# codebits1001/CET-driven-simulation-for-3D-printing-AM-KMC-Approach

Hardware: AMD Instinct MI355X
Metric: kmc_events_per_sec (higher is better)
Workload: dtype f64

## Files before the change

cet-driven-simulation-for-3d-printing-am-kmc-approach_amd/cetkmc/_lib.py:

```python
import ctypes as C
import glob
import os
import subprocess

_HERE = os.path.dirname(os.path.abspath(__file__))
CSRC = os.path.join(os.path.dirname(_HERE), "csrc")
INCLUDE = os.path.join(os.path.dirname(os.path.dirname(_HERE)), "include")
SO_PATH = os.path.join(CSRC, "libcetkmc_hip.so")


def sources():
    return sorted(glob.glob(os.path.join(CSRC, "*.hip")) + glob.glob(os.path.join(CSRC, "*.hpp")) +
                  glob.glob(os.path.join(INCLUDE, "*.h")))


HIPCC_FLAGS = ["--offload-arch=gfx950", "-O3", "-std=c++17", "-fPIC", "-shared", "-ffp-contract=off",
               "-fno-fast-math", "-I/opt/rocm/include"]


class Params(C.Structure):
    _fields_ = [
        ("nu", C.c_double), ("nu_dep", C.c_double), ("E_b", C.c_double * 3), ("E_diff", C.c_double * 3),
        ("kT", C.c_double), ("T_melt", C.c_double), ("I0", C.c_double), ("delta_T_c", C.c_double),
        ("K_nuc", C.c_double), ("beta_imp_nuc", C.c_double), ("max_imp_frac", C.c_double),
# ... 99 lines not shown
        ("n_bins", C.c_int32), ("pad", C.c_int32), ("gb_edges", C.POINTER(C.c_double)), ("pole_edges", C.POINTER(C.c_double)),
        ("axis", C.c_double * 3),
    ]


class SolidInfo(C.Structure):
    _fields_ = [("n_new", C.c_int64), ("n_cleared", C.c_int64), ("n_recorded", C.c_int64)]


class SolidArgs(C.Structure):
    _fields_ = [("qscale", C.c_double * 4)]


class SolidRec(C.Structure):
    _fields_ = [("n_rec", C.c_int64), ("n_bad", C.c_int64), ("n_cooling", C.c_int64), ("stamp_sum", C.c_int64),
                ("stamp_min", C.c_int64), ("stamp_max", C.c_int64), ("q", C.c_int64 * 4)]


STRUCT_MIRRORS = {"params": Params, "event": Event, "sweep_info": SweepInfo, "run_args": RunArgs, "run_result": RunResult,
                  "super_args": SuperArgs, "counters": Counters, "host_comm": HostComm, "ens_args": EnsArgs,
                  "ens_analysis": EnsAnalysis, "front_stats": FrontStats, "layer_rec": LayerRec,
                  "texture_args": TextureArgs, "grain_rec": GrainRec, "solid_info": SolidInfo, "solid_args": SolidArgs,
                  "solid_rec": SolidRec}

_P = C.POINTER
PROTOTYPES = {
    "cetkmc_last_error": (C.c_char_p, []),
    "cetkmc_abi_version": (C.c_int, []),
    "cetkmc_source_hash": (C.c_char_p, []),
    "cetkmc_struct_size": (C.c_int, [C.c_char_p]),
    "cetkmc_dirty_offset": (C.c_int, [C.c_int, C.c_int]),
    "cetkmc_stale_row": (C.c_int, [C.c_int, _P(C.c_int), _P(C.c_int), C.c_int, C.c_int]),
    "cetkmc_stale_rows": (C.c_int, [C.c_int, _P(C.c_int), _P(C.c_int), C.c_int, C.c_void_p]),
    "cetkmc_device_count": (C.c_int, [_P(C.c_int)]),
    "cetkmc_create": (C.c_int, [_P(Params), C.c_int, C.c_int, _P(C.c_int), _P(C.c_void_p)]),
    "cetkmc_get_unique_id": (C.c_int, [C.c_char_p]),
    "cetkmc_create_rank": (C.c_int, [_P(Params), C.c_int, C.c_int, C.c_int, C.c_int, C.c_char_p, _P(C.c_void_p)]),
    "cetkmc_create_rank_host": (C.c_int, [_P(Params), C.c_int, C.c_int, C.c_int, C.c_int, _P(HostComm), _P(C.c_void_p)]),
    "cetkmc_destroy": (C.c_int, [C.c_void_p]),
    "cetkmc_set_params": (C.c_int, [C.c_void_p, _P(Params)]),
    "cetkmc_sync": (C.c_int, [C.c_void_p]),
    "cetkmc_set_option": (C.c_int, [C.c_void_p, C.c_char_p, C.c_int64]),
    "cetkmc_owned_planes": (C.c_int, [C.c_void_p, _P(C.c_int), _P(C.c_int)]),
    "cetkmc_upload": (C.c_int, [C.c_void_p, C.c_void_p, C.c_void_p, C.c_void_p, C.c_void_p, C.c_void_p]),
    "cetkmc_download": (C.c_int, [C.c_void_p, C.c_void_p, C.c_void_p, C.c_void_p, C.c_void_p, C.c_void_p]),
    "cetkmc_upload_planes": (C.c_int, [C.c_void_p, C.c_int, C.c_int, C.c_void_p, C.c_void_p, C.c_void_p, C.c_void_p, C.c_void_p]),
    "cetkmc_download_planes": (C.c_int, [C.c_void_p, C.c_int, C.c_int, C.c_void_p, C.c_void_p, C.c_void_p, C.c_void_p, C.c_void_p]),
    "cetkmc_set_defects": (C.c_int, [C.c_void_p, C.c_void_p]),
    "cetkmc_set_prev_state": (C.c_int, [C.c_void_p, C.c_void_p]),
    "cetkmc_thermal_cet": (C.c_int, [C.c_void_p, C.c_double, C.c_int]),
    "cetkmc_thermal_laser": (C.c_int, [C.c_void_p, C.c_double, C.c_void_p, C.c_int, C.c_int]),
    "cetkmc_rate_sweep": (C.c_int, [C.c_void_p, _P(SweepInfo)]),
    "cetkmc_select": (C.c_int, [C.c_void_p, C.c_double, _P(Event)]),
    "cetkmc_apply": (C.c_int, [C.c_void_p, _P(Event), C.c_double, C.c_double, C.c_int]),
    "cetkmc_enumerate_events": (C.c_int, [C.c_void_p, C.c_void_p, C.c_int64, _P(C.c_int64)]),
    "cetkmc_row_sums": (C.c_int, [C.c_void_p, C.c_void_p, C.c_void_p]),
    "cetkmc_run_steps": (C.c_int, [C.c_void_p, _P(RunArgs), _P(RunResult), C.c_void_p, C.c_void_p, C.c_void_p]),
    "cetkmc_stage_inputs": (C.c_int, [C.c_void_p, _P(RunArgs)]),
    "cetkmc_run_supersteps": (C.c_int, [C.c_void_p, _P(SuperArgs), _P(RunResult), C.c_void_p, C.c_void_p, C.c_void_p, C.c_void_p]),
    "cetkmc_get_counters": (C.c_int, [C.c_void_p, _P(Counters), C.c_int]),
    "cetkmc_cluster": (C.c_int, [C.c_void_p, C.c_double, _P(C.c_int64)]),
    "cetkmc_cluster_stats": (C.c_int, [C.c_void_p, C.c_int64, C.c_void_p, C.c_void_p, C.c_void_p]),
    "cetkmc_cluster_labels": (C.c_int, [C.c_void_p, C.c_void_p]),
    "cetkmc_species_counts": (C.c_int, [C.c_void_p, C.c_void_p]),
    "cetkmc_gather_species": (C.c_int, [C.c_void_p, C.c_int, C.c_void_p, C.c_void_p, C.c_int64, _P(C.c_int64)]),
    "cetkmc_set_defects_sparse": (C.c_int, [C.c_void_p, C.c_void_p, C.c_int64]),
# ... 123 lines not shown
```

cet-driven-simulation-for-3d-printing-am-kmc-approach_amd/csrc/cetkmc_hip.hip:

```cpp
#include <dlfcn.h>
#include <hip/hip_runtime.h>
#include <hip/hip_ext.h>
#include <rccl/rccl.h>

#include <algorithm>
#include <chrono>
#include <cmath>
#include <cstdint>
#include <climits>
#include <cstdio>
#include <cstring>
#include <map>
#include <mutex>
#include <string>
#include <type_traits>
#include <vector>

#include "kernels.hpp"
#include "cluster.hpp"
#include "superstep.hpp"
#include "ensemble.hpp"
#include "front.hpp"
#include "layer.hpp"
#include "texture.hpp"
// ... 78 lines not shown
#define NCCLCHK(expr)                                                                             \
    do {                                                                                          \
        ncclResult_t r_ = (expr);                                                                 \
        if (r_ != ncclSuccess)                                                                    \
            return fail(std::string(#expr) + ": " + g_rccl.GetErrorString(r_));                   \
    } while (0)

struct Slab {
    SlabView v{};
    uint8_t* prev = nullptr;
    double* Tbuf[2] = {nullptr, nullptr};
    double* vvalbuf[2] = {nullptr, nullptr};
    double* depbuf[2] = {nullptr, nullptr};
    size_t nS = 0, nT = 0, nC = 0;
};

struct Handle {
    cetkmc_params p{};
    KParams kp{};
    int L = 0, Pk = 1, PB = 1, RJ = 0, pitchS = 0, pitchT = 0, pitchC = 0;
    int dev = 0;
    hipStream_t stream = nullptr, stream2 = nullptr;
    std::vector<Slab> slabs;
    SlabView* d_views[2] = {nullptr, nullptr};
    int cur = 0;
    int G = 1, my_first = 0;
    int own_i0 = 0, own_i1 = 0;
    BlockEnt* d_blocks = nullptr;
    cetkmc_event* d_events_all = nullptr;
    StepState* d_ss = nullptr;
    int* d_dirty = nullptr;
    PendRec* d_pend = nullptr;
    int apply_in_sweep = 1;
    bool pend_live = false;
    BatchCfg pend_cfg{};
    double* d_ktab = nullptr;
    KParams* d_kp = nullptr;
    void* d_scratch = nullptr;
    size_t scratch_bytes = 0;
    int* d_flag = nullptr;
    double* d_qtop = nullptr;
    double *d_u_pick = nullptr, *d_u_defect = nullptr, *d_u_np = nullptr, *d_q = nullptr, *d_log_total = nullptr;
    cetkmc_event* d_log_event = nullptr;
    int64_t* d_log_nev = nullptr;
    size_t cap_steps = 0, cap_np = 0, cap_q = 0;
    char* pin_in = nullptr; size_t pin_in_cap = 0;
    char* pin_out = nullptr; size_t pin_out_cap = 0;
    struct { bool valid = false, has_defect = false; int64_t step0 = 0, n_steps = 0, np_cap = 0, n_q = 0; int thermal_mode = 0; } staged;
    ncclComm_t comm = nullptr;
    int rank = 0, nranks = 1;
    bool swept = false;
    int sweep_auto = 1;
    int sweep_variant = 1;
    bool table_fresh = false;
    bool ifc_fresh = false;
    int ifc_every_step = 0;
    int thermal_variant = 1;
    int thermal_general = 0;
    int therm_ni = THERM_NI;
    int therm_ni16 = THERM16_NI;
    int thermal_rpt = 2;
    int thermal_kt = 256;
    int thermal_tiles16 = 1;
    int ifc_blocks = 64;
    int ifc_block = 256;
    size_t shmem_stream = 0;
// ... 459 lines not shown
    HIPCHK(hipMemcpyAsync(buf, host, per * h->nranks, hipMemcpyHostToDevice, h->stream));
    HIPCHK(hipStreamSynchronize(h->stream));
    return 0;
}
int comm_allgather(Handle* h, void* buf, size_t per)
{
    CHK(comm_stamp(h));
    CHK(comm_allgather_raw(h, buf, per));
    return comm_stamp(h);
}

int launch_dirty_rows(Handle* h, hipEvent_t ev_a, hipEvent_t ev_b)
{
    if (ev_a) HIPCHK(hipEventRecord(ev_a, h->stream));
    for (size_t s = 0; s < h->slabs.size(); ++s) {
        SlabView v = view_of(h, (int)s);
        const StreamArgs sa = stream_args(h, v);
        const int* dl = h->d_dirty;
        int* pc = h->d_dirty + 1 + DIRTY_MAX;
        const StepState* ss = h->d_ss;
        with_rows(row_shape(h), [&](auto hw, auto ch2) {
            with_flag(h->sweep_variant == 1 || h->sweep_variant >= 3, [&](auto tab) {
                launch(k_rows_eval<tab.value, hw.value, ch2.value>, dim3(24), dim3(256), 0, h->stream, nullptr, nullptr, sa, dl, ss, h->d_blocks, pc);
            });
        });
    }
    if (ev_b) HIPCHK(hipEventRecord(ev_b, h->stream));
    HIPCHK(hipGetLastError());
    if (multi_rank(h)) CHK(comm_allgather(h, h->d_blocks, (size_t)3 * (h->L / h->nranks) * sizeof(BlockEnt)));
    h->swept = true;
    return 0;
}

int launch_sweep(Handle* h, bool batch, hipEvent_t ev_a = nullptr, hipEvent_t ev_b = nullptr, bool long_list = false,
                 hipEvent_t ev_pre = nullptr, hipEvent_t ev_post = nullptr)
{
    ++h->cnt.sweeps;
    for (auto& sl : h->slabs) h->cnt.alg_bytes_sweep += (int64_t)9 * sl.v.nloc * h->L * h->L;
    if (ev_pre) HIPCHK(hipEventRecord(ev_pre, h->stream));
    const int TR = SWEEP_TJ + 4;
    const size_t shmem0 = (size_t)((5 * TR * h->pitchS + 15) & ~15) + 225 * sizeof(double);
    const StepState* ss = batch ? h->d_ss : nullptr;
    const int njt = (h->L + SWEEP_TJ - 1) / SWEEP_TJ;
    if (h->sweep_variant >= 1) {
        if (h->pend_live && (!h->table_fresh || !h->ifc_fresh)) return fail("internal: rate table / interface sums stale under a pending event");
        CHK(ensure_table(h, h->stream, ss));
        if (!h->ifc_fresh || h->ifc_every_step) {
            CHK(launch_interface(h, batch, h->stream, long_list));
            ++h->cnt.interface_launches;
            h->ifc_fresh = true;
        }
    }
    const bool ext = ev_a && ev_b && !ev_pre && h->slabs.size() == 1 && h->sweep_variant >= 1;
    const hipEvent_t xa = ext ? ev_a : nullptr, xb = ext ? ev_b : nullptr;
    if (ev_a && !ext) HIPCHK(hipEventRecord(ev_a, h->stream));
    const int sv = (h->sweep_auto && h->sweep_variant == 1 && h->L <= 128) ? 4 : h->sweep_variant;
    const RowShape rs = row_shape(h);
    for (size_t s = 0; s < h->slabs.size(); ++s) {
        SlabView v = view_of(h, (int)s);
        const StreamArgs sa = stream_args(h, v);
        if (sv == 4) {
            with_rows(rs, [&](auto hw, auto ch2) {
                launch(k_sweep_plane<hw.value, ch2.value>, dim3((unsigned)v.nloc), dim3(1024), plane_shmem(h->L), h->stream, xa, xb, sa, ss, h->d_blocks);
            });
        } else if (sv == 3) {
            const int ipp = rs.hw ? (h->L + 1) / 2 : h->L;
            const int64_t n_items = (int64_t)ipp * v.nloc;
            const dim3 g((unsigned)((n_items + 4 * TABLE_IPW - 1) / (4 * TABLE_IPW)));
            with_rows(rs, [&](auto hw, auto ch2) {
                launch(k_sweep_table<hw.value, ch2.value>, g, dim3(256), 0, h->stream, xa, xb, sa, ss);
            });
        } else if (h->sweep_variant >= 1 && h->pend_live) {
            ApplyArgs X{h->kp, (const SlabView*)h->d_views[h->cur], h->d_pend, h->d_ss, h->pend_cfg, (const double*)h->d_u_defect,
                        (const double*)h->d_u_np, (const double*)h->d_ktab, h->d_log_total, h->d_log_event, h->d_log_nev};
            launch(k_sweep_stream_apply<true, 1, false>, dim3(sa.group_count * njt + 1), dim3(256), h->shmem_stream, h->stream, xa, xb, sa, h->d_ss, X);
        } else if (h->sweep_variant >= 1) {
            auto go = [&](auto k) { launch(k, dim3(sa.group_count * njt), dim3(256), h->shmem_stream, h->stream, xa, xb, sa, ss); };
            if (h->sweep_variant == 1) with_stream_kernel<true>(rs, go); else with_stream_kernel<false>(rs, go);
        } else {
            hipLaunchKernelGGL(k_sweep_simple, dim3(v.nloc * njt), dim3(256), shmem0, h->stream, h->kp, v, h->d_ktab, ss);
        }
    }
    if (ev_b && !ext) HIPCHK(hipEventRecord(ev_b, h->stream));
    if (sv != 4)
        for (size_t s = 0; s < h->slabs.size(); ++s) {
            SlabView v = view_of(h, (int)s);
            hipLaunchKernelGGL(k_plane_reduce, dim3(3 * v.nloc), dim3(64), 0, h->stream, v, h->d_blocks, ss);
        }
    HIPCHK(hipGetLastError());
    if (multi_rank(h)) CHK(comm_allgather(h, h->d_blocks, (size_t)3 * (h->L / h->nranks) * sizeof(BlockEnt)));
    if (ev_post) HIPCHK(hipEventRecord(ev_post, h->stream));
    h->swept = true;
    return 0;
}

int launch_select(Handle* h, const BatchCfg& cfg, double r_direct, int info_only)
{
    hipLaunchKernelGGL(k_select, dim3(1), dim3(256), 0, h->stream, h->kp, (const SlabView*)h->d_views[h->cur],
                       (int)h->slabs.size(), h->L, h->PB, (const BlockEnt*)h->d_blocks, h->d_ss, cfg,
                       (const double*)h->d_u_pick, r_direct, (const double*)h->d_ktab,
                       h->d_events_all + h->my_first, info_only, h->sweep_variant >= 1 ? 1 : 0);
    HIPCHK(hipGetLastError());
    if (multi_rank(h) && !info_only) CHK(comm_allgather(h, h->d_events_all, sizeof(cetkmc_event)));
    return 0;
}

int launch_select_apply(Handle* h, const BatchCfg& cfg, int eval_touched, int* dirty, int64_t cur_hint)
{
// ... 381 lines not shown
const char* cetkmc_last_error(void) { return g_err.c_str(); }
int cetkmc_abi_version(void) { return CETKMC_ABI_VERSION; }
#ifndef CETKMC_SRC_HASH
#define CETKMC_SRC_HASH "unknown"
#endif
static const char g_src_hash[] = "cetkmc-source-hash=" CETKMC_SRC_HASH;
const char* cetkmc_source_hash(void) { return g_src_hash + 19; }

int cetkmc_struct_size(const char* name)
{
    if (!name) return -1;
#define SZ(n, t) if (!strcmp(name, n)) return (int)sizeof(t)
    SZ("params", cetkmc_params); SZ("event", cetkmc_event); SZ("sweep_info", cetkmc_sweep_info);
    SZ("run_args", cetkmc_run_args); SZ("run_result", cetkmc_run_result); SZ("super_args", cetkmc_super_args);
    SZ("counters", cetkmc_counters); SZ("host_comm", cetkmc_host_comm); SZ("ens_args", cetkmc_ens_args); SZ("ens_analysis", cetkmc_ens_analysis);
    SZ("front_stats", struct cetkmc_front_stats); SZ("layer_rec", struct cetkmc_layer_rec); SZ("texture_args", struct cetkmc_texture_args);
    SZ("grain_rec", struct cetkmc_grain_rec);
    SZ("solid_info", struct cetkmc_solid_info); SZ("solid_args", struct cetkmc_solid_args); SZ("solid_rec", struct cetkmc_solid_rec);
#undef SZ
    return -1;
}

int cetkmc_dirty_offset(int di, int dj) { return dirty_offset(di, dj) ? 1 : 0; }
static StaleEv stale_ev_host(int type, const int pos[2], const int target[2])
{
    StaleEv se;
    se.type = type; se.pi = pos[0]; se.pj = pos[1]; se.ti = target[0]; se.tj = target[1];
    return se;
}
int cetkmc_stale_row(int type, const int pos[2], const int target[2], int gi, int j)
{
    return stale_row(stale_ev_host(type, pos, target), gi, j) ? 1 : 0;
}
int cetkmc_stale_rows(int type, const int pos[2], const int target[2], int L, int rows[][2])
{
    const StaleEv se = stale_ev_host(type, pos, target);
    int n = 0;
    for (int c = 0; c < STALE_CAND; ++c) {
        int gi, j;
        if (!stale_candidate(se, L, c, gi, j)) continue;
        if (n < PATCH_MAX) { rows[n][0] = gi; rows[n][1] = j; }
        ++n;
    }
    return n;
}

int cetkmc_device_count(int* n)
{
    if (!n) return fail("null argument");
    int c = 0;
    hipError_t e = hipGetDeviceCount(&c);
    if (e != hipSuccess) { *n = 0; return fail(std::string("hipGetDeviceCount: ") + hipGetErrorString(e)); }
    *n = c;
    return 0;
}

int cetkmc_create(const cetkmc_params* p, int L, int n_slabs, const int* device_ids, void** handle)
{
    if (n_slabs < 1) return fail("n_slabs must be >= 1");
    int dev = device_ids ? device_ids[0] : 0;
    for (int s = 1; s < n_slabs && device_ids; ++s)
        if (device_ids[s] != dev)
            return fail("in-process slabs must share one device; multi-GPU runs use one process per GPU (cetkmc_create_rank)");
    if (n_slabs > 1 && L / n_slabs < 2) return fail("each slab needs at least 2 planes");
    std::vector<std::pair<int, int>> ranges;
    int base = L / n_slabs, rem = L % n_slabs, at = 0;
// ... 65 lines not shown
{
    Handle* h = (Handle*)handle;
    if (!h || !p) return fail("null argument");
    HIPCHK(hipSetDevice(h->dev));
    h->p = *p; h->kp = make_kparams(*p);
    h->swept = false; h->table_fresh = false; h->ifc_fresh = false;
    return upload_ktab(h);
}

int cetkmc_set_option(void* handle, const char* key, int64_t value)
{
    Handle* h = (Handle*)handle;
    if (!h || !key) return fail("null argument");
    if (!strcmp(key, "sweep_variant")) {
        if (value < 0 || value > 4) return fail("sweep_variant must be 0 (simple), 1 (streaming + rate table, default), 2 (streaming, recompute), 3 (census-free table sweep) or 4 (census-free, one block per plane, block sums in the same launch)");
        h->sweep_variant = (int)value;
        h->sweep_auto = 0;
        h->swept = false; h->table_fresh = false; h->ifc_fresh = false;
        return 0;
    }
    if (!strcmp(key, "interface_every_step")) { h->ifc_every_step = value ? 1 : 0; h->ifc_fresh = false; return 0; }
    if (!strcmp(key, "thermal_planes_per_block")) {
        if (value < 1 || value > 64) return fail("thermal_planes_per_block must be 1..64");
        h->therm_ni = (int)value;
        return 0;
    }
    if (!strcmp(key, "thermal_planes_per_block16")) {
        if (value < 1 || value > 64) return fail("thermal_planes_per_block16 must be 1..64");
        h->therm_ni16 = (int)value;
        return 0;
    }
    if (!strcmp(key, "thermal_lookahead")) { h->thermal_ahead = value ? 1 : 0; return 0; }
    if (!strcmp(key, "apply_in_sweep")) { h->apply_in_sweep = value ? 1 : 0; return 0; }
    if (!strcmp(key, "thermal_table")) { h->thermal_table = value ? 1 : 0; return 0; }
    if (!strcmp(key, "reserve_batch")) {
        if (value < 0 || value > (1 << 22)) return fail("reserve_batch out of range");
        HIPCHK(hipSetDevice(h->dev));
        h->staged.valid = false;
        const size_t n = (size_t)value;
        CHK(reserve_steps(h, n));
        CHK(grow(&h->d_u_np, &h->cap_np, 2 * n + 2 + (size_t)h->L * h->L));
        CHK(grow(&h->d_q, &h->cap_q, (n / 20 + 2) * (size_t)h->L * h->L));
        CHK(grow_pinned(&h->pin_in, &h->pin_in_cap, 2 * n * 8 + (2 * n + 2) * 8 + std::min<size_t>(PIN_SMALL_MAX, (n / 20 + 2) * (size_t)h->L * h->L * 8)));
        CHK(grow_pinned(&h->pin_out, &h->pin_out_cap, 64 + n * (16 + sizeof(cetkmc_event)) + h->slabs.size() * sizeof(int)));
        return reserve_events(h, std::max<int64_t>(7 * std::min<int64_t>(value, 256), value <= 64 ? 2 * value : 2 * (value / 8 + 1)));
    }
    if (!strcmp(key, "thermal_variant")) {
        if (value < 0 || value > 5) return fail("thermal_variant must be 0 (simple), 1 (marching, default: 16-row tiles, 2 rows per thread), 2 (marching, general kernel only), 3 (16-row tiles, 4 rows per thread), 4 (8-row tiles) or 5 (16-row x 128-column tiles)");
        h->thermal_general = value == 2 ? 1 : 0;
        h->thermal_tiles16 = value == 4 ? 0 : 1;
        h->thermal_rpt = value == 3 ? 4 : 2;
        h->thermal_kt = value == 5 ? 128 : 256;
        if (value >= 2) value = 1;
        h->thermal_variant = (int)value;
        return 0;
    }
    return fail(std::string("unknown option ") + key);
}

int cetkmc_sync(void* handle)
{
    Handle* h = (Handle*)handle;
    if (!h) return fail("null handle");
    HIPCHK(hipStreamSynchronize(h->stream));
    return 0;
}
// ... 1897 lines not shown
```

cet-driven-simulation-for-3d-printing-am-kmc-approach_amd/csrc/kernels.hpp:

```cpp
#pragma once
#include "voxel.hpp"
#include "../../include/cetkmc.h"

namespace cetkmc {

struct BlockEnt { double sum; int64_t cnt; };

struct StepState {
    int64_t cur;
    int32_t status;
    int32_t pad0;
    int64_t np_pos;
    int64_t nuc_count;
    double  total;
    int64_t n_events;
    int64_t n_dep;
    double  min_margin;
};

template <class S> __device__ __forceinline__ const auto& ens_rep(unsigned r, const S& sel) { return sel.reps[r]; }
template <class S> __device__ __forceinline__ int ens_rel(const S& sel) { return sel.rel; }
template <class S> __device__ __forceinline__ unsigned ens_nz(const S& sel) { return (unsigned)sel.nz; }
template <class S> __device__ __forceinline__ int64_t ens_stride(const S& sel) { return sel.stride; }
template <class S> __device__ __forceinline__ const long long* ens_offs(const S& sel) { return sel.offs; }
// ... 555 lines not shown
            {
                load_vals<TAB, HW>(A, li, j0 + row_of(1), lane, 0, nxt);
                const int r = row_of(0);
                auto rowp = [&](int d, int dj) { return (const uint8_t*)smem + so[d + 2] + (r + 2 + dj) * pitchC + KOFFC; };
                sweep_row<TAB, HW, CH2, SK>(A, rowp, li, lp, j0 + r, top, lane, cur, sw);
            }
            {
#ifdef CETKMC_NO_TAIL_PREFETCH
                if (more)
#endif
                load_vals<TAB, HW>(A, min(li + 1, lp1 + 1), j0 + row_of(0), lane, 0, cur);
                const int r = row_of(1);
                auto rowp = [&](int d, int dj) { return (const uint8_t*)smem + so[d + 2] + (r + 2 + dj) * pitchC + KOFFC; };
                sweep_row<TAB, HW, CH2, SK>(A, rowp, li, lp, j0 + r, top, lane, nxt, sw);
            }
        }
#ifdef CETKMC_NO_TAIL_PREFETCH
        if (more)
#endif
        store_slab(li + 3);
        __syncthreads();
    };
    if (NP == 1) {
#pragma unroll 1
        for (int lp = lp0; lp < lp1; lp += 2) {
            plane(lp, va, vb);
            if (lp + 1 < lp1) plane(lp + 1, vb, va);
        }
    } else {
#pragma unroll 1
        for (int lp = lp0; lp < lp1; ++lp) plane(lp, va, vb);
    }
}
template <bool TAB, bool HW, int NPF, bool CH2>
__global__ __launch_bounds__(256) CETKMC_SWEEP_ATTR void k_sweep_stream(StreamArgs A, const StepState* __restrict__ ss)
{
    if (ss && ss->status) return;
    extern __shared__ __attribute__((aligned(16))) unsigned char smem[];
    sweep_stream_tile<TAB, HW, NPF, CH2>(A, blockIdx.x, smem);
}

__device__ __forceinline__ uint2 load_cls8(const StreamArgs& A, int li, int jrow, int sl, int m)
{
    const int k0 = min((m << 9) + 8 * sl, A.pitchT - 8);
    const int jr = min(jrow, A.L - 1);
    return *reinterpret_cast<const uint2*>(A.cls + ((int64_t)li * A.RJ + (jr + 2)) * A.pitchC + KOFFC + k0);
}
template <bool HW, bool CH2>
__device__ __forceinline__ void table_row(const StreamArgs& A, int li, int lp, int jrow, bool top, int lane, const double (&v0)[8],
                                          uint2 own0, double* lds_sum = nullptr, int* lds_cnt = nullptr )
{
    static_assert(!(HW && CH2), "half-wave rows have one chunk");
    const int L = A.L;
    const int sl = HW ? (lane & 31) : lane;
    constexpr int nch = CH2 ? 2 : 1;
    double r0 = 0.0, r1 = 0.0, r2 = 0.0;
    int nE_a = 0, nE_b = 0, nD_a = 0, nD_b = 0;
    int cI = 0;
    bool any_ifc = false;
#pragma unroll
    for (int m = 0; m < nch; ++m) {
        const int k0 = (m << 9) + 8 * sl;
        const bool active = jrow < L && k0 < L;
        double v[8], ev[8];
        uint2 own = own0;
        if (m == 0) {
#pragma unroll
            for (int q = 0; q < 8; ++q) v[q] = v0[q];
        } else {
            load_vals<true, HW>(A, li, jrow, lane, m, v);
            own = load_cls8(A, li, jrow, sl, m);
        }
        if (!active) own = make_uint2(0u, 0u);
        const uint2 E = make_uint2(own.x & 0x01010101u, own.y & 0x01010101u);
        const uint2 Aat = make_uint2((own.x >> 1) & 0x01010101u, (own.y >> 1) & 0x01010101u);
        const uint2 c6 = make_uint2((own.x >> 2) & 0x3F3F3F3Fu, (own.y >> 2) & 0x3F3F3F3Fu);
#pragma unroll
        for (int h = 0; h < 8; ++h) ev[h] = mask_f64(v[h], h < 4 ? E.x : E.y, 8 * (h & 3));
        const uint2 cE = make_uint2(c6.x & (E.x * 255u), c6.y & (E.y * 255u));
        const uint2 cA = make_uint2(c6.x & (Aat.x * 255u), c6.y & (Aat.y * 255u));
        const bool diff_here = __any((cA.x | cA.y) != 0u);
        double dv[8];
#pragma unroll
// ... 20 lines not shown
        r2 = (m == 0) ? s2 : r2 + s2;
        double s1 = 0.0;
        if (diff_here) s1 = wave_tree_sum_h<HW>(tree8(dv));
        r1 = (m == 0) ? s1 : r1 + s1;
        if (top) {
            double dp[8];
#pragma unroll
            for (int q = 0; q < 8; ++q) dp[q] = 0.0;
            if (active) {
                const double2* src = reinterpret_cast<const double2*>(A.dep_val + (int64_t)jrow * A.pitchT + k0);
#pragma unroll
                for (int q = 0; q < 4; ++q) { const double2 t = src[q]; dp[2 * q] = t.x; dp[2 * q + 1] = t.y; }
            }
#pragma unroll
            for (int h = 0; h < 8; ++h) {
                const bool keep = (((h < 4 ? E.x : E.y) >> (8 * (h & 3))) & 1u) && finite_d(dp[h]);
                dp[h] = keep ? dp[h] : 0.0;
                const unsigned long long bm = __ballot(keep);
                if (HW) { nD_a += __popc((unsigned)bm); nD_b += __popc((unsigned)(bm >> 32)); }
                else nD_a += __popcll(bm);
            }
            const double s0 = wave_tree_sum_h<HW>(tree8(dp));
            r0 = (m == 0) ? s0 : r0 + s0;
        }
    }
    int n2 = HW ? ((lane & 32) ? nE_b : nE_a) : nE_a;
    const int n0 = HW ? ((lane & 32) ? nD_b : nD_a) : nD_a;
    int n1 = 0;
    if (any_ifc) {
        const int packed = wave_sum_i_h<HW>(cI);
        n2 += packed & 0xFFFF;
        n1 = packed >> 16;
    }
    if (sl == 0 && jrow < L) {
        const int64_t o = (int64_t)lp * 3 * L + jrow;
        A.rowsum[o] = r0; A.rowsum[o + L] = r1; A.rowsum[o + 2 * (int64_t)L] = r2;
        A.rowcnt[o] = n0; A.rowcnt[o + L] = n1; A.rowcnt[o + 2 * (int64_t)L] = n2;
        if (lds_sum) {
            lds_sum[jrow] = r0; lds_sum[L + jrow] = r1; lds_sum[2 * L + jrow] = r2;
            lds_cnt[jrow] = n0; lds_cnt[L + jrow] = n1; lds_cnt[2 * L + jrow] = n2;
        }
    }
}

#ifndef CETKMC_TABLE_IPW
#define CETKMC_TABLE_IPW 8
#endif
constexpr int TABLE_IPW = CETKMC_TABLE_IPW;
template <bool HW, bool CH2>
__global__ __launch_bounds__(256) CETKMC_SWEEP_ATTR void k_sweep_table(StreamArgs A, const StepState* __restrict__ ss)
{
    if (ss && ss->status) return;
    const int tid = threadIdx.x, lane = tid & 63, w = tid >> 6;
    const int L = A.L;
    const int ipp = HW ? (L + 1) >> 1 : L;
    const int n_items = ipp * A.nloc;
    int b = blockIdx.x;
    if ((gridDim.x & 7) == 0) b = (b & 7) * (int)(gridDim.x >> 3) + (b >> 3);
    int item = b * 4 * TABLE_IPW + w;
    if (item >= n_items) return;
    int lp = item / ipp, jp = item - lp * ipp;
    const int sl = HW ? (lane & 31) : lane;
    auto jrow_of = [&](int jpair) { return HW ? 2 * jpair + (lane >> 5) : jpair; };
#ifdef CETKMC_TABLE_DEPTH2
    double va[8], vb[8], vc[8];
    uint2 ca, cb, cc;
    auto advance = [&](int& lpx, int& jpx) { jpx += 4; while (jpx >= ipp) { jpx -= ipp; ++lpx; } };
    int lp1 = lp, jp1 = jp;
    advance(lp1, jp1);
    const bool has1 = item + 4 < n_items;
    load_vals<true, HW>(A, lp + 2, jrow_of(jp), lane, 0, va);
    ca = load_cls8(A, lp + 2, jrow_of(jp), sl, 0);
    load_vals<true, HW>(A, (has1 ? lp1 : lp) + 2, jrow_of(has1 ? jp1 : jp), lane, 0, vb);
    cb = load_cls8(A, (has1 ? lp1 : lp) + 2, jrow_of(has1 ? jp1 : jp), sl, 0);
    int done = 0;
    auto step = [&](double (&cur)[8], uint2& ccur, double (&far)[8], uint2& cfar) {
        int lp2 = lp, jp2 = jp;
        advance(lp2, jp2);
        int lp3 = lp2, jp3 = jp2;
        advance(lp3, jp3);
        const bool more = (done + 2 < TABLE_IPW) && (item + 8 < n_items);
        load_vals<true, HW>(A, (more ? lp3 : lp) + 2, jrow_of(more ? jp3 : jp), lane, 0, far);
        cfar = load_cls8(A, (more ? lp3 : lp) + 2, jrow_of(more ? jp3 : jp), sl, 0);
        table_row<HW, CH2>(A, lp + 2, lp, jrow_of(jp), A.gi0 + lp == L - 1, lane, cur, ccur);
        item += 4; lp = lp2; jp = jp2; ++done;
    };
#pragma unroll 1
    while (true) {
        step(va, ca, vc, cc);
        if (done >= TABLE_IPW || item >= n_items) break;
        step(vb, cb, va, ca);
        if (done >= TABLE_IPW || item >= n_items) break;
        step(vc, cc, vb, cb);
        if (done >= TABLE_IPW || item >= n_items) break;
    }
#else
    double va[8], vb[8];
    uint2 ca, cb;
    load_vals<true, HW>(A, lp + 2, jrow_of(jp), lane, 0, va);
    ca = load_cls8(A, lp + 2, jrow_of(jp), sl, 0);
    auto step = [&](double (&cur)[8], uint2& ccur, double (&nxt)[8], uint2& cnxt, bool last) {
        int lp2 = lp, jp2 = jp + 4;
        while (jp2 >= ipp) { jp2 -= ipp; ++lp2; }
        const bool more = !last && (item + 4 < n_items);
        const int lpn = more ? lp2 : lp, jpn = more ? jp2 : jp;
        load_vals<true, HW>(A, lpn + 2, jrow_of(jpn), lane, 0, nxt);
        cnxt = load_cls8(A, lpn + 2, jrow_of(jpn), sl, 0);
        table_row<HW, CH2>(A, lp + 2, lp, jrow_of(jp), A.gi0 + lp == L - 1, lane, cur, ccur);
        item += 4; lp = lp2; jp = jp2;
    };
#pragma unroll 1
    for (int t = 0; t < TABLE_IPW; t += 2) {
        step(va, ca, vb, cb, false);
        if (item >= n_items) break;
        step(vb, cb, va, ca, t + 2 >= TABLE_IPW);
        if (item >= n_items) break;
    }
#endif
}

template <bool HW, bool CH2, class... E>
__global__ __launch_bounds__(1024) CETKMC_SWEEP_ATTR void k_sweep_plane(StreamArgs A, const StepState* __restrict__ ss, BlockEnt* __restrict__ blocks, E... ens)
{
    if constexpr (sizeof...(E) > 0) {
        const auto& e = ens_rep(blockIdx.y, ens...);
        A = e.sa[ens_rel(ens...)]; ss = e.ss; blocks = e.blocks;
    }
    if (ss && ss->status) return;
    extern __shared__ __attribute__((aligned(16))) unsigned char smem[];
    const int tid = threadIdx.x, lane = tid & 63, w = tid >> 6;
    const int L = A.L;
    double* lds_sum = reinterpret_cast<double*>(smem);
    int* lds_cnt = reinterpret_cast<int*>(lds_sum + 3 * L);
    const int ipp = HW ? (L + 1) >> 1 : L;
    int lp = blockIdx.x;
    if ((gridDim.x & 7) == 0) lp = (lp & 7) * (int)(gridDim.x >> 3) + (lp >> 3);
    const int sl = HW ? (lane & 31) : lane;
    auto jrow_of = [&](int jpair) { return HW ? 2 * jpair + (lane >> 5) : jpair; };
    const bool top = A.gi0 + lp == L - 1;
    int jp = w;
    if (jp < ipp) {
        double va[8], vb[8];
        uint2 ca, cb;
        load_vals<true, HW>(A, lp + 2, jrow_of(jp), lane, 0, va);
        ca = load_cls8(A, lp + 2, jrow_of(jp), sl, 0);
        auto step = [&](double (&cur)[8], uint2& ccur, double (&nxt)[8], uint2& cnxt) {
            const int jpn = (jp + 16 < ipp) ? jp + 16 : jp;
            load_vals<true, HW>(A, lp + 2, jrow_of(jpn), lane, 0, nxt);
            cnxt = load_cls8(A, lp + 2, jrow_of(jpn), sl, 0);
            table_row<HW, CH2>(A, lp + 2, lp, jrow_of(jp), top, lane, cur, ccur, lds_sum, lds_cnt);
// ... 981 lines not shown
    for (int q = threadIdx.x; q < (int)(sizeof(SlabView) / 8); q += blockDim.x)
        reinterpret_cast<uint64_t*>(Sl)[q] = reinterpret_cast<const uint64_t*>(X.slabs)[q];
    __syncthreads();
    apply_batch_body<PEND_EB>(*Pl, Sl, 1, A.L, &X.pend->ev, 1, X.ss, X.cfg, X.u_defect, X.u_np, X.log_total, X.log_event, X.log_nev,
                              X.ktab_g, 1, nullptr, &X.pend->carry);
#ifdef CETKMC_SEL_STAMPS
    if (threadIdx.x == 0) g_pend_stamps[1] = g_sel_stamps[10];
#endif
    __builtin_amdgcn_fence(__ATOMIC_RELEASE, "agent");
    __syncthreads();
    __builtin_amdgcn_fence(__ATOMIC_ACQUIRE, "agent");
    PEND_STAMP(2);
    const StaleEv se = stale_ev_of(X.pend->ev);
    const int lane = threadIdx.x & 63, w = __builtin_amdgcn_readfirstlane((int)(threadIdx.x >> 6)), L = A.L;
    int cgi = 0, cj = 0;
    unsigned long long m = __ballot(lane < STALE_CAND && stale_candidate(se, L, lane, cgi, cj));
    for (int k = w; k > 0; --k) m &= m - 1;
    while (m) {
        int gi, j;
        stale_candidate_row(se, __builtin_ctzll(m), gi, j);
        const int lp = gi - A.gi0, li = lp + 2;
        const int jrow = (HW && lane >= 32) ? L_INACTIVE : j;
        double v0[8];
        load_vals<true, HW>(A, li, jrow, lane, 0, v0);
        table_row<HW, CH2>(A, li, lp, jrow, gi == L - 1, lane, v0, load_cls8(A, li, jrow, HW ? (lane & 31) : lane, 0));
        for (int k = 4; k > 0; --k) m &= m - 1;
    }
#ifdef CETKMC_SEL_STAMPS
    __syncthreads();
    PEND_STAMP(3);
#endif
}

template <bool HW, int NPF, bool CH2>
__global__ __launch_bounds__(256) __attribute__((amdgpu_waves_per_eu(5))) void k_sweep_stream_apply(StreamArgs A,
                                                                                                    const StepState* __restrict__ ss,
                                                                                                    ApplyArgs X)
{
    if (ss->status) return;
    extern __shared__ __attribute__((aligned(16))) unsigned char smem[];
    if (blockIdx.x != 0) {
        const int b = (int)blockIdx.x - 1;
        const StaleEv se = stale_ev_of(X.pend->ev);
        int ibr, jt;
        stream_tile_of(A, b, ibr, jt);
        const int g0 = A.gi0 + (A.group_first + ibr) * STREAM_NI, j0 = jt * SWEEP_TJ;
        auto meets = [&](int ci, int cj) {
            return ci + 2 >= g0 && ci - 2 < g0 + STREAM_NI && cj + 2 >= j0 && cj - 2 < j0 + SWEEP_TJ;
        };
        if (se.type >= 0 && (meets(se.pi, se.pj) || (se.type == EV_DIFF && meets(se.ti, se.tj))))
            sweep_stream_tile<true, HW, NPF, CH2, true>(A, b, smem, stale_win(se));
        else
            sweep_stream_tile<true, HW, NPF, CH2>(A, b, smem);
#ifdef CETKMC_SEL_STAMPS
        if (threadIdx.x == 0) atomicMax(&g_pend_stamps[4], (unsigned long long)wall_clock64());
#endif
        return;
    }
    sweep_apply_block<HW, CH2>(A, X, smem);
}

__global__ __launch_bounds__(64) void k_apply_direct(KParams P, const SlabView* __restrict__ slabs, int nslabs, cetkmc_event ev,
                                                     int make_defect, StepState* ss, const double* __restrict__ ktab_g)
{
    if (threadIdx.x == 0) {
        if (ev.type == EV_NUC) ss->nuc_count += 1;
        apply_event(slabs, nslabs, ev, make_defect);
    }
    __syncthreads();
    apply_touch(P, slabs, nslabs, ktab_g, ev, threadIdx.x, 0, blockDim.x);
}

__global__ void k_empty() {}

template <class... E>
__global__ void k_batch_reset(StepState* ss, E... ens)
{
    if constexpr (sizeof...(E) > 0) {
        const auto& e = ens_rep(blockIdx.x, ens...);
        ss = e.ss;
        if (!e.active) { ss->cur = 0; ss->status = 1; ss->np_pos = 0; ss->min_margin = 1.0; return; }
    }
    ss->cur = 0; ss->status = 0; ss->np_pos = 0; ss->min_margin = 1.0;
}

struct ThermalCfg {
// ... 564 lines not shown
```

include/cetkmc.h:

```cpp
#ifndef CETKMC_H
#define CETKMC_H

#include <stdint.h>

#ifdef __cplusplus
extern "C" {
#endif

#define CETKMC_ABI_VERSION 1

typedef struct cetkmc_params {
    double nu;
    double nu_dep;
    double E_b[3];
    double E_diff[3];
    double kT;
    double T_melt;
    double I0;
    double delta_T_c;
    double K_nuc;
    double beta_imp_nuc;
    double max_imp_frac;
    double rate_threshold;
    double anisotropy;
// ... 68 lines not shown
    int32_t thermal_mode;
    double  thermal_dt;
    const double* q_planes;
    int64_t n_q;
    int32_t use_latent;
    int32_t null_events;
} cetkmc_super_args;

typedef struct cetkmc_counters {
    int64_t steps;
    int64_t sweeps;
    int64_t incremental_steps;
    int64_t thermal_updates;
    int64_t supersteps;
    int64_t bytes_h2d, bytes_d2h;
    int64_t alg_bytes_sweep, alg_bytes_thermal;
    int64_t profiled_steps;
    double  ms_thermal, ms_interface , ms_sweep, ms_dirty_rows, ms_reduce, ms_select_apply;
    int64_t alg_bytes_table;
    int64_t table_updates;
    int64_t interface_launches;
    double  ms_comm;
    int64_t comm_calls;
    int64_t deferred_steps;
} cetkmc_counters;

const char* cetkmc_last_error(void);
int cetkmc_abi_version(void);
const char* cetkmc_source_hash(void);
int cetkmc_struct_size(const char* name);
int cetkmc_dirty_offset(int di, int dj);
int cetkmc_stale_row(int type, const int pos[2], const int target[2], int gi, int j);
int cetkmc_stale_rows(int type, const int pos[2], const int target[2], int L, int rows[][2]);
int cetkmc_device_count(int* n);

int cetkmc_create(const cetkmc_params* p, int L, int n_slabs, const int* device_ids, void** handle);
int cetkmc_get_unique_id(char out[128]);
int cetkmc_create_rank(const cetkmc_params* p, int L, int rank, int nranks, int device_id,
                       const char unique_id[128], void** handle);
typedef int (*cetkmc_allgather_fn)(void* user, const void* send, void* recv, int64_t nbytes);
typedef int (*cetkmc_exchange_fn)(void* user, int lo, int hi, const void* send_lo, void* recv_lo, const void* send_hi,
                                  void* recv_hi, int64_t nbytes);
typedef struct cetkmc_host_comm {
    cetkmc_allgather_fn allgather;
    cetkmc_exchange_fn exchange;
    void* user;
} cetkmc_host_comm;
int cetkmc_create_rank_host(const cetkmc_params* p, int L, int rank, int nranks, int device_id, const cetkmc_host_comm* hc,
                            void** handle);
int cetkmc_destroy(void* handle);
int cetkmc_set_params(void* handle, const cetkmc_params* p);
int cetkmc_sync(void* handle);
int cetkmc_set_option(void* handle, const char* key, int64_t value);
int cetkmc_owned_planes(void* handle, int* i0, int* i1);

int cetkmc_upload(void* handle, const int64_t* state, const double* theta, const double* phi,
                  const double* T, const int64_t* defects);
int cetkmc_download(void* handle, int64_t* state, double* theta, double* phi, double* T,
                    int64_t* defects);
int cetkmc_upload_planes(void* handle, int i_begin, int i_end, const uint8_t* state,
                         const double* theta, const double* phi, const double* T,
                         const uint8_t* defects);
int cetkmc_download_planes(void* handle, int i_begin, int i_end, uint8_t* state, double* theta,
                           double* phi, double* T, uint8_t* defects);
int cetkmc_set_defects(void* handle, const uint8_t* mask);
int cetkmc_set_prev_state(void* handle, const int64_t* prev_state);
// ... 143 lines not shown
```

Before: 17020.

## Use census-free table tiles in the pending-event sweep-apply launch

Adds a table-tile sweep path that assigns row items to waves in a flat, interleaved order with double-buffered loads. It reads from the rate table instead of using ring-shaped shared-memory stream tiles. The fused sweep+apply kernel uses this path by default for single-slab, single-rank runs with L>128 and half-wave rows, skipping rowsum writes for rows made stale by the pending event. The aim is to drop shared-memory staging and the per-tile stale-window checks, and to spread work across more, smaller blocks. The risk is lower reuse of neighbor data, and the path only runs at particular shapes.

```diff
diff --git a/cet-driven-simulation-for-3d-printing-am-kmc-approach_amd/cetkmc/_lib.py b/cet-driven-simulation-for-3d-printing-am-kmc-approach_amd/cetkmc/_lib.py
--- a/cet-driven-simulation-for-3d-printing-am-kmc-approach_amd/cetkmc/_lib.py
+++ b/cet-driven-simulation-for-3d-printing-am-kmc-approach_amd/cetkmc/_lib.py
@@ -155,6 +155,7 @@
     "cetkmc_dirty_offset": (C.c_int, [C.c_int, C.c_int]),
     "cetkmc_stale_row": (C.c_int, [C.c_int, _P(C.c_int), _P(C.c_int), C.c_int, C.c_int]),
     "cetkmc_stale_rows": (C.c_int, [C.c_int, _P(C.c_int), _P(C.c_int), C.c_int, C.c_void_p]),
+    "cetkmc_table_tile_of": (C.c_int, [C.c_int, C.c_int, C.c_int]),
     "cetkmc_device_count": (C.c_int, [_P(C.c_int)]),
     "cetkmc_create": (C.c_int, [_P(Params), C.c_int, C.c_int, _P(C.c_int), _P(C.c_void_p)]),
     "cetkmc_get_unique_id": (C.c_int, [C.c_char_p]),
diff --git a/cet-driven-simulation-for-3d-printing-am-kmc-approach_amd/csrc/cetkmc_hip.hip b/cet-driven-simulation-for-3d-printing-am-kmc-approach_amd/csrc/cetkmc_hip.hip
--- a/cet-driven-simulation-for-3d-printing-am-kmc-approach_amd/csrc/cetkmc_hip.hip
+++ b/cet-driven-simulation-for-3d-printing-am-kmc-approach_amd/csrc/cetkmc_hip.hip
@@ -134,6 +134,7 @@
     int* d_dirty = nullptr;
     PendRec* d_pend = nullptr;
     int apply_in_sweep = 1;
+    int fused_tiles = 1;
     bool pend_live = false;
     BatchCfg pend_cfg{};
     double* d_ktab = nullptr;
@@ -659,6 +660,12 @@
     return 0;
 }
 
+bool table_tiles(const Handle* h, int level)
+{
+    return h->fused_tiles >= level && h->slabs.size() == 1 && !multi_rank(h) && h->L > 128 && row_shape(h).hw;
+}
+size_t apply_shmem() { return ((sizeof(KParams) + 15) & ~(size_t)15) + sizeof(SlabView); }
+
 int launch_sweep(Handle* h, bool batch, hipEvent_t ev_a = nullptr, hipEvent_t ev_b = nullptr, bool long_list = false,
                  hipEvent_t ev_pre = nullptr, hipEvent_t ev_post = nullptr)
 {
@@ -700,7 +707,12 @@
         } else if (h->sweep_variant >= 1 && h->pend_live) {
             ApplyArgs X{h->kp, (const SlabView*)h->d_views[h->cur], h->d_pend, h->d_ss, h->pend_cfg, (const double*)h->d_u_defect,
                         (const double*)h->d_u_np, (const double*)h->d_ktab, h->d_log_total, h->d_log_event, h->d_log_nev};
-            launch(k_sweep_stream_apply<true, 1, false>, dim3(sa.group_count * njt + 1), dim3(256), h->shmem_stream, h->stream, xa, xb, sa, h->d_ss, X);
+            if (table_tiles(h, 1))
+                launch(k_sweep_stream_apply<true, 1, false, true>, dim3(table_tile_count(h->L, v.nloc, true) + 1), dim3(256), apply_shmem(), h->stream, xa, xb, sa, h->d_ss, X);
+            else
+                launch(k_sweep_stream_apply<true, 1, false>, dim3(sa.group_count * njt + 1), dim3(256), h->shmem_stream, h->stream, xa, xb, sa, h->d_ss, X);
+        } else if (h->sweep_variant == 1 && table_tiles(h, 2)) {
+            launch(k_sweep_stream<true, true, 1, false, true>, dim3(table_tile_count(h->L, v.nloc, true)), dim3(256), 0, h->stream, xa, xb, sa, ss);
         } else if (h->sweep_variant >= 1) {
             auto go = [&](auto k) { launch(k, dim3(sa.group_count * njt), dim3(256), h->shmem_stream, h->stream, xa, xb, sa, ss); };
             if (h->sweep_variant == 1) with_stream_kernel<true>(rs, go); else with_stream_kernel<false>(rs, go);
@@ -1148,6 +1160,11 @@
 {
     return stale_row(stale_ev_host(type, pos, target), gi, j) ? 1 : 0;
 }
+int cetkmc_table_tile_of(int L, int gi, int j)
+{
+    if (L <= 128 || L > 256 || gi < 0 || gi >= L || j < 0 || j >= L) return -1;
+    return table_tile_of(L, true, gi, j);
+}
 int cetkmc_stale_rows(int type, const int pos[2], const int target[2], int L, int rows[][2])
 {
     const StaleEv se = stale_ev_host(type, pos, target);
@@ -1279,6 +1296,11 @@
     }
     if (!strcmp(key, "thermal_lookahead")) { h->thermal_ahead = value ? 1 : 0; return 0; }
     if (!strcmp(key, "apply_in_sweep")) { h->apply_in_sweep = value ? 1 : 0; return 0; }
+    if (!strcmp(key, "fused_tiles")) {
+        if (value < 0 || value > 2) return fail("fused_tiles must be 0 (ring tiles), 1 (census-free tiles in the launch that applies a pending event, default) or 2 (in the plain streaming launch at that shape as well)");
+        h->fused_tiles = (int)value;
+        return 0;
+    }
     if (!strcmp(key, "thermal_table")) { h->thermal_table = value ? 1 : 0; return 0; }
     if (!strcmp(key, "reserve_batch")) {
         if (value < 0 || value > (1 << 22)) return fail("reserve_batch out of range");
diff --git a/cet-driven-simulation-for-3d-printing-am-kmc-approach_amd/csrc/kernels.hpp b/cet-driven-simulation-for-3d-printing-am-kmc-approach_amd/csrc/kernels.hpp
--- a/cet-driven-simulation-for-3d-printing-am-kmc-approach_amd/csrc/kernels.hpp
+++ b/cet-driven-simulation-for-3d-printing-am-kmc-approach_amd/csrc/kernels.hpp
@@ -611,13 +611,6 @@
         for (int lp = lp0; lp < lp1; ++lp) plane(lp, va, vb);
     }
 }
-template <bool TAB, bool HW, int NPF, bool CH2>
-__global__ __launch_bounds__(256) CETKMC_SWEEP_ATTR void k_sweep_stream(StreamArgs A, const StepState* __restrict__ ss)
-{
-    if (ss && ss->status) return;
-    extern __shared__ __attribute__((aligned(16))) unsigned char smem[];
-    sweep_stream_tile<TAB, HW, NPF, CH2>(A, blockIdx.x, smem);
-}
 
 __device__ __forceinline__ uint2 load_cls8(const StreamArgs& A, int li, int jrow, int sl, int m)
 {
@@ -625,9 +618,10 @@
     const int jr = min(jrow, A.L - 1);
     return *reinterpret_cast<const uint2*>(A.cls + ((int64_t)li * A.RJ + (jr + 2)) * A.pitchC + KOFFC + k0);
 }
-template <bool HW, bool CH2>
+template <bool HW, bool CH2, bool SK = false>
 __device__ __forceinline__ void table_row(const StreamArgs& A, int li, int lp, int jrow, bool top, int lane, const double (&v0)[8],
-                                          uint2 own0, double* lds_sum = nullptr, int* lds_cnt = nullptr )
+                                          uint2 own0, double* lds_sum = nullptr, int* lds_cnt = nullptr ,
+                                          const StaleWin& sw = StaleWin{})
 {
     static_assert(!(HW && CH2), "half-wave rows have one chunk");
     const int L = A.L;
@@ -714,7 +708,7 @@
         n2 += packed & 0xFFFF;
         n1 = packed >> 16;
     }
-    if (sl == 0 && jrow < L) {
+    if (sl == 0 && jrow < L && !(SK && stale_row(sw, A.gi0 + lp, jrow))) {
         const int64_t o = (int64_t)lp * 3 * L + jrow;
         A.rowsum[o] = r0; A.rowsum[o + L] = r1; A.rowsum[o + 2 * (int64_t)L] = r2;
         A.rowcnt[o] = n0; A.rowcnt[o + L] = n1; A.rowcnt[o + 2 * (int64_t)L] = n2;
@@ -729,10 +723,76 @@
 #define CETKMC_TABLE_IPW 8
 #endif
 constexpr int TABLE_IPW = CETKMC_TABLE_IPW;
+
+#ifndef CETKMC_TILE_IPW
+#define CETKMC_TILE_IPW 2
+#endif
+constexpr int TABLE_TILE_IPW = CETKMC_TILE_IPW;
+constexpr int TABLE_TILE_ITEMS = 4 * TABLE_TILE_IPW;
+__host__ __device__ constexpr int table_tile_ipp(int L, bool hw) { return hw ? (L + 1) >> 1 : L; }
+__host__ __device__ constexpr int table_tile_count(int L, int nloc, bool hw)
+{
+    return (table_tile_ipp(L, hw) * nloc + TABLE_TILE_ITEMS - 1) / TABLE_TILE_ITEMS;
+}
+__host__ __device__ constexpr int table_tile_of(int L, bool hw, int lp, int j)
+{
+    return (lp * table_tile_ipp(L, hw) + (hw ? j >> 1 : j)) / TABLE_TILE_ITEMS;
+}
+template <bool HW, bool CH2, bool SK, int IPW>
+__device__ __forceinline__ void sweep_table_tile(const StreamArgs& A, int b, int nblk, const StaleWin& sw = StaleWin{})
+{
+    static_assert(IPW % 2 == 0, "two alternating buffers");
+    const int tid = threadIdx.x, lane = tid & 63, w = __builtin_amdgcn_readfirstlane(tid >> 6);
+    const int L = A.L;
+    const int ipp = table_tile_ipp(L, HW);
+    const int n_items = ipp * A.nloc;
+    if ((nblk & 7) == 0) b = (b & 7) * (nblk >> 3) + (b >> 3);
+    int item = b * 4 * IPW + w;
+    if (item >= n_items) return;
+    int lp = item / ipp, jp = item - lp * ipp;
+    const int sl = HW ? (lane & 31) : lane;
+    auto jrow_of = [&](int jpair) { return HW ? 2 * jpair + (lane >> 5) : jpair; };
+    double va[8], vb[8];
+    uint2 ca, cb;
+    load_vals<true, HW>(A, lp + 2, jrow_of(jp), lane, 0, va);
+    ca = load_cls8(A, lp + 2, jrow_of(jp), sl, 0);
+    auto step = [&](double (&cur)[8], uint2& ccur, double (&nxt)[8], uint2& cnxt, bool last) {
+        int lp2 = lp, jp2 = jp + 4;
+        while (jp2 >= ipp) { jp2 -= ipp; ++lp2; }
+        const bool more = !last && (item + 4 < n_items);
+        const int lpn = more ? lp2 : lp, jpn = more ? jp2 : jp;
+        load_vals<true, HW>(A, lpn + 2, jrow_of(jpn), lane, 0, nxt);
+        cnxt = load_cls8(A, lpn + 2, jrow_of(jpn), sl, 0);
+        table_row<HW, CH2, SK>(A, lp + 2, lp, jrow_of(jp), A.gi0 + lp == L - 1, lane, cur, ccur, nullptr, nullptr, sw);
+        item += 4; lp = lp2; jp = jp2;
+    };
+#pragma unroll 1
+    for (int t = 0; t < IPW; t += 2) {
+        step(va, ca, vb, cb, false);
+        if (item >= n_items) break;
+        step(vb, cb, va, ca, t + 2 >= IPW);
+        if (item >= n_items) break;
+    }
+}
+
+template <bool TAB, bool HW, int NPF, bool CH2, bool TT = false>
+__global__ __launch_bounds__(256) CETKMC_SWEEP_ATTR void k_sweep_stream(StreamArgs A, const StepState* __restrict__ ss)
+{
+    static_assert(!TT || TAB, "census-free tiles read the rate table");
+    if (ss && ss->status) return;
+    if constexpr (TT) {
+        sweep_table_tile<HW, CH2, false, TABLE_TILE_IPW>(A, blockIdx.x, (int)gridDim.x);
+    } else {
+        extern __shared__ __attribute__((aligned(16))) unsigned char smem[];
+        sweep_stream_tile<TAB, HW, NPF, CH2>(A, blockIdx.x, smem);
+    }
+}
+
 template <bool HW, bool CH2>
 __global__ __launch_bounds__(256) CETKMC_SWEEP_ATTR void k_sweep_table(StreamArgs A, const StepState* __restrict__ ss)
 {
     if (ss && ss->status) return;
+#ifdef CETKMC_TABLE_DEPTH2
     const int tid = threadIdx.x, lane = tid & 63, w = tid >> 6;
     const int L = A.L;
     const int ipp = HW ? (L + 1) >> 1 : L;
@@ -744,7 +804,6 @@
     int lp = item / ipp, jp = item - lp * ipp;
     const int sl = HW ? (lane & 31) : lane;
     auto jrow_of = [&](int jpair) { return HW ? 2 * jpair + (lane >> 5) : jpair; };
-#ifdef CETKMC_TABLE_DEPTH2
     double va[8], vb[8], vc[8];
     uint2 ca, cb, cc;
     auto advance = [&](int& lpx, int& jpx) { jpx += 4; while (jpx >= ipp) { jpx -= ipp; ++lpx; } };
@@ -777,27 +836,7 @@
         if (done >= TABLE_IPW || item >= n_items) break;
     }
 #else
-    double va[8], vb[8];
-    uint2 ca, cb;
-    load_vals<true, HW>(A, lp + 2, jrow_of(jp), lane, 0, va);
-    ca = load_cls8(A, lp + 2, jrow_of(jp), sl, 0);
-    auto step = [&](double (&cur)[8], uint2& ccur, double (&nxt)[8], uint2& cnxt, bool last) {
-        int lp2 = lp, jp2 = jp + 4;
-        while (jp2 >= ipp) { jp2 -= ipp; ++lp2; }
-        const bool more = !last && (item + 4 < n_items);
-        const int lpn = more ? lp2 : lp, jpn = more ? jp2 : jp;
-        load_vals<true, HW>(A, lpn + 2, jrow_of(jpn), lane, 0, nxt);
-        cnxt = load_cls8(A, lpn + 2, jrow_of(jpn), sl, 0);
-        table_row<HW, CH2>(A, lp + 2, lp, jrow_of(jp), A.gi0 + lp == L - 1, lane, cur, ccur);
-        item += 4; lp = lp2; jp = jp2;
-    };
-#pragma unroll 1
-    for (int t = 0; t < TABLE_IPW; t += 2) {
-        step(va, ca, vb, cb, false);
-        if (item >= n_items) break;
-        step(vb, cb, va, ca, t + 2 >= TABLE_IPW);
-        if (item >= n_items) break;
-    }
+    sweep_table_tile<HW, CH2, false, TABLE_IPW>(A, blockIdx.x, (int)gridDim.x);
 #endif
 }
 
@@ -1845,7 +1884,7 @@
 #endif
 }
 
-template <bool HW, int NPF, bool CH2>
+template <bool HW, int NPF, bool CH2, bool TT = false>
 __global__ __launch_bounds__(256) __attribute__((amdgpu_waves_per_eu(5))) void k_sweep_stream_apply(StreamArgs A,
                                                                                                     const StepState* __restrict__ ss,
                                                                                                     ApplyArgs X)
@@ -1855,16 +1894,20 @@
     if (blockIdx.x != 0) {
         const int b = (int)blockIdx.x - 1;
         const StaleEv se = stale_ev_of(X.pend->ev);
-        int ibr, jt;
-        stream_tile_of(A, b, ibr, jt);
-        const int g0 = A.gi0 + (A.group_first + ibr) * STREAM_NI, j0 = jt * SWEEP_TJ;
-        auto meets = [&](int ci, int cj) {
-            return ci + 2 >= g0 && ci - 2 < g0 + STREAM_NI && cj + 2 >= j0 && cj - 2 < j0 + SWEEP_TJ;
-        };
-        if (se.type >= 0 && (meets(se.pi, se.pj) || (se.type == EV_DIFF && meets(se.ti, se.tj))))
-            sweep_stream_tile<true, HW, NPF, CH2, true>(A, b, smem, stale_win(se));
-        else
-            sweep_stream_tile<true, HW, NPF, CH2>(A, b, smem);
+        if constexpr (TT) {
+            sweep_table_tile<HW, CH2, true, TABLE_TILE_IPW>(A, b, (int)gridDim.x - 1, stale_win(se));
+        } else {
+            int ibr, jt;
+            stream_tile_of(A, b, ibr, jt);
+            const int g0 = A.gi0 + (A.group_first + ibr) * STREAM_NI, j0 = jt * SWEEP_TJ;
+            auto meets = [&](int ci, int cj) {
+                return ci + 2 >= g0 && ci - 2 < g0 + STREAM_NI && cj + 2 >= j0 && cj - 2 < j0 + SWEEP_TJ;
+            };
+            if (se.type >= 0 && (meets(se.pi, se.pj) || (se.type == EV_DIFF && meets(se.ti, se.tj))))
+                sweep_stream_tile<true, HW, NPF, CH2, true>(A, b, smem, stale_win(se));
+            else
+                sweep_stream_tile<true, HW, NPF, CH2>(A, b, smem);
+        }
 #ifdef CETKMC_SEL_STAMPS
         if (threadIdx.x == 0) atomicMax(&g_pend_stamps[4], (unsigned long long)wall_clock64());
 #endif
diff --git a/include/cetkmc.h b/include/cetkmc.h
--- a/include/cetkmc.h
+++ b/include/cetkmc.h
@@ -124,6 +124,7 @@
 int cetkmc_dirty_offset(int di, int dj);
 int cetkmc_stale_row(int type, const int pos[2], const int target[2], int gi, int j);
 int cetkmc_stale_rows(int type, const int pos[2], const int target[2], int L, int rows[][2]);
+int cetkmc_table_tile_of(int L, int gi, int j);
 int cetkmc_device_count(int* n);
 
 int cetkmc_create(const cetkmc_params* p, int L, int n_slabs, const int* device_ids, void** handle);
```

New measurement: 18000 (median of 6 runs). +5.8%, better.
